# WeiZhang1988/YDORBSLAM

Measured on AMD Instinct MI355X. Metric: ORB extract+match Mkeypoints/sec, higher is better.
Workload: dtype u8

## Files before the change

ydorbslam_amd/csrc/extract_kernels.hip.h:

```cpp
#pragma once
#include <hip/hip_runtime.h>
#include <stdint.h>

#include "quadtree_core.h"
#include "quadtree_flat.h"

#pragma clang fp contract(off)

namespace ydorb {

constexpr int kPad = 19;
constexpr int kBorder = 16;
constexpr int kMaxLevels = 8;
constexpr int kTileMax = 72;
#ifndef QT_THREADS
#define QT_THREADS 512
#endif
constexpr int kQtThreads = QT_THREADS;

struct LevelDev {
  int w, h, pitch;
  int padOff;
  int blurOff, blurPitch;
  int cellBegin, nCells;
  int quota;
  int candOff;
  int kpOff;
  int tabOff;
  int nodeTabOff;
  float scale;
  float size;
};
struct PlanDev {
  int nLevels, nCellsTotal, cellCap, sumQuota;
  int maxX[16];
  unsigned nodeTabFrameStride;
  int blurTileBegin[kMaxLevels + 1];
  int borderBegin[kMaxLevels + 1];
  LevelDev lv[kMaxLevels];
};
#ifndef BLUR_TH
#define BLUR_TH 58
#endif
constexpr int kBlurTW = 64, kBlurTH = BLUR_TH;
struct CellDev {
  short level, x0, y0, x1, y1, pad0;
  int srcOff;
};

__device__ __forceinline__ int reflect101(int i, int n) {
  if (n == 1) return 0;
  while (i < 0 || i >= n) i = i < 0 ? -i : 2 * (n - 1) - i;
  return i;
}

typedef uint32_t __attribute__((aligned(1))) u32_unaligned;
typedef unsigned long long __attribute__((aligned(1))) u64_unaligned;

#ifndef PYR_ROWS
#define PYR_ROWS 8
#endif
constexpr int kPyrRows = PYR_ROWS;
__global__ __launch_bounds__(256) void k_pyr_level0(const uint8_t* __restrict__ img, int stride, size_t frameStride,
                                                    uint8_t* __restrict__ pyr, size_t pyrFrameStride, LevelDev L) {
  const int wx = blockIdx.x * 64 + (threadIdx.x & 63);
  const int yb = (blockIdx.y * 4 + __builtin_amdgcn_readfirstlane(threadIdx.x >> 6)) * kPyrRows;
  const int x0 = wx * 4 - kPad;
  if (x0 + 3 < 0 || x0 >= L.w) return;
  const uint8_t* src = img + (size_t)blockIdx.z * frameStride;
  uint8_t* dst = pyr + (size_t)blockIdx.z * pyrFrameStride + L.padOff + (size_t)kPad * L.pitch + wx * 4;
  const int xa = L.w >= 4 ? min(max(x0, 0), L.w - 4) : 0, sh = 8 * (x0 - xa);
  uint32_t v[kPyrRows];
#pragma unroll
  for (int r = 0; r < kPyrRows; r++) {
    const uint8_t* row = src + (size_t)min(yb + r, L.h - 1) * stride;
    if (L.w >= 4) {
      v[r] = *reinterpret_cast<const u32_unaligned*>(row + xa);
    } else {
      v[r] = 0;
      for (int b = 0; b < L.w; b++) v[r] |= (uint32_t)row[b] << (8 * b);
    }
    v[r] = sh < 0 ? v[r] << (-sh) : v[r] >> sh;
  }
#pragma unroll
  for (int r = 0; r < kPyrRows; r++)
    if (yb + r < L.h) *reinterpret_cast<uint32_t*>(dst + (size_t)(yb + r) * L.pitch) = v[r];
}

__global__ __launch_bounds__(256) void k_pyr_resize(uint8_t* __restrict__ pyr, size_t pyrFrameStride, LevelDev Lp, LevelDev L,
                                                    double scaleX, const short* __restrict__ alpha,
                                                    const int* __restrict__ yofs, const short* __restrict__ beta) {
  const int wx = blockIdx.x * 64 + (threadIdx.x & 63);
  const int yb = (blockIdx.y * 4 + __builtin_amdgcn_readfirstlane(threadIdx.x >> 6)) * kPyrRows;
  const int x0 = wx * 4 - kPad;
  if (x0 + 3 < 0 || x0 >= L.w) return;
  uint8_t* frame = pyr + (size_t)blockIdx.z * pyrFrameStride;
  const uint8_t* S = frame + Lp.padOff + (size_t)kPad * Lp.pitch + kPad;
  uint8_t* dst = frame + L.padOff + (size_t)kPad * L.pitch + wx * 4;
  int sx[4], sx1[4], a0[4], a1[4];
#pragma unroll
  for (int b = 0; b < 4; b++) {
    const int dx = min(max(x0 + b, 0), L.w - 1);
    const float fx = (float)__dsub_rn(__dmul_rn((double)dx + 0.5, scaleX), 0.5);
    sx[b] = min(max((int)floorf(fx), 0), Lp.w - 1);
    a0[b] = alpha[2 * dx]; a1[b] = alpha[2 * dx + 1];
    sx1[b] = min(sx[b] + 1, Lp.w - 1);
  }
  const bool fast = sx[3] - sx[0] <= 6;
  const uint8_t *r0p[kPyrRows], *r1p[kPyrRows];
  int b0[kPyrRows], b1[kPyrRows];
#pragma unroll
  for (int r = 0; r < kPyrRows; r++) {
    const int dy = min(yb + r, L.h - 1);
    const int sy = yofs[dy];
    b0[r] = beta[2 * dy]; b1[r] = beta[2 * dy + 1];
    r0p[r] = S + (size_t)min(max(sy, 0), Lp.h - 1) * Lp.pitch;
    r1p[r] = S + (size_t)min(max(sy + 1, 0), Lp.h - 1) * Lp.pitch;
  }
  uint32_t v[kPyrRows];
  if (fast) {
    typedef unsigned short u16x2 __attribute__((ext_vector_type(2)));
    uint32_t sel[4];
    u16x2 ab[4];
#pragma unroll
    for (int b = 0; b < 4; b++) {
      const uint32_t off = (uint32_t)(sx[b] - sx[0]);
      sel[b] = off | 0x0c000c00u | ((off + 1) << 16);
      ab[b] = u16x2{(unsigned short)a0[b], (unsigned short)a1[b]};
    }
    unsigned long long w0[kPyrRows], w1[kPyrRows];
#pragma unroll
    for (int r = 0; r < kPyrRows; r++) {
      w0[r] = *reinterpret_cast<const u64_unaligned*>(r0p[r] + sx[0]);
      w1[r] = *reinterpret_cast<const u64_unaligned*>(r1p[r] + sx[0]);
    }
#pragma unroll
    for (int r = 0; r < kPyrRows; r++) {
      v[r] = 0;
#pragma unroll
      for (int b = 0; b < 4; b++) {
        const uint32_t p0 = __builtin_amdgcn_perm((uint32_t)(w0[r] >> 32), (uint32_t)w0[r], sel[b]);
        const uint32_t p1 = __builtin_amdgcn_perm((uint32_t)(w1[r] >> 32), (uint32_t)w1[r], sel[b]);
        const int h0 = (int)__builtin_amdgcn_udot2(__builtin_bit_cast(u16x2, p0), ab[b], 0u, false);
        const int h1 = (int)__builtin_amdgcn_udot2(__builtin_bit_cast(u16x2, p1), ab[b], 0u, false);
        const int o = (((b0[r] * (h0 >> 4)) >> 16) + ((b1[r] * (h1 >> 4)) >> 16) + 2) >> 2;
        v[r] |= (uint32_t)(o & 0xFF) << (8 * b);
      }
    }
  } else {
#pragma unroll
    for (int r = 0; r < kPyrRows; r++) {
      v[r] = 0;
#pragma unroll
      for (int b = 0; b < 4; b++) {
        const int h0 = r0p[r][sx[b]] * a0[b] + r0p[r][sx1[b]] * a1[b];
        const int h1 = r1p[r][sx[b]] * a0[b] + r1p[r][sx1[b]] * a1[b];
        const int o = (((b0[r] * (h0 >> 4)) >> 16) + ((b1[r] * (h1 >> 4)) >> 16) + 2) >> 2;
        v[r] |= (uint32_t)(o & 0xFF) << (8 * b);
      }
    }
  }
#pragma unroll
  for (int r = 0; r < kPyrRows; r++)
    if (yb + r < L.h) *reinterpret_cast<uint32_t*>(dst + (size_t)(yb + r) * L.pitch) = v[r];
}

struct PyrPadEntry { uint32_t laneA4, laneB4, selM, selF; };
struct PyrColEntry { uint32_t sel[4]; uint32_t ab[4]; };
constexpr uint32_t kPermIdentity = 0x03020100u;
#ifndef PYR_ROWS_F
#define PYR_ROWS_F 8
#endif
constexpr int kPyrRowsF = PYR_ROWS_F;

__device__ __forceinline__ uint32_t pyr_finish_dword(uint32_t v, const PyrPadEntry& pe) {
  const uint32_t A = (uint32_t)__builtin_amdgcn_ds_bpermute((int)pe.laneA4, (int)v);
  const uint32_t B = (uint32_t)__builtin_amdgcn_ds_bpermute((int)pe.laneB4, (int)v);
  const uint32_t M = __builtin_amdgcn_perm(A, B, pe.selM);
  return __builtin_amdgcn_perm(M, v, pe.selF);
}
__device__ __forceinline__ void pyr_store_rows(uint8_t* dst, int pitch, int y, int h, uint32_t v) {
  if (y >= h) return;
  *reinterpret_cast<uint32_t*>(dst + (ptrdiff_t)y * pitch) = v;
  if (y >= 1 && y <= kPad) *reinterpret_cast<uint32_t*>(dst - (ptrdiff_t)y * pitch) = v;
  if (y >= h - 1 - kPad && y <= h - 2) *reinterpret_cast<uint32_t*>(dst + (ptrdiff_t)(2 * (h - 1) - y) * pitch) = v;
}

__global__ __launch_bounds__(256) void k_pyr_level0_f(const uint8_t* __restrict__ img, int stride, size_t frameStride,
                                                      uint8_t* __restrict__ pyr, size_t pyrFrameStride, LevelDev L,
                                                      const PyrPadEntry* __restrict__ padTab, int shift) {
  const int wx = blockIdx.x * 64 + (threadIdx.x & 63) - shift;
  const int yb = (blockIdx.y * 4 + __builtin_amdgcn_readfirstlane(threadIdx.x >> 6)) * kPyrRowsF;
  const int nd = (L.w + 2 * kPad + 3) >> 2;
  if (wx < 0 || wx >= nd) return;
  const int x0 = wx * 4 - kPad;
  const uint8_t* src = img + (size_t)blockIdx.z * frameStride;
  uint8_t* dst = pyr + (size_t)blockIdx.z * pyrFrameStride + L.padOff + (size_t)kPad * L.pitch + wx * 4;
// ... 794 lines not shown
#pragma unroll
      for (int jj = 0; jj < 4; jj++) { key[jj] = (int)(st[4 * g + jj] & 0xFFFu); slot[jj] = qf_off(Pn) + (key[jj] >> (2 * (D - Pn))); }
      for (int d = Pn - 1; d >= 1; d--) {
        const int off = qf_off(d), sh = 2 * (D - d);
#pragma unroll
        for (int jj = 0; jj < 4; jj++) {
          const int sl = off + (key[jj] >> sh);
          if (hist[sl] == 1) slot[jj] = sl;
        }
      }
#pragma unroll
      for (int jj = 0; jj < 4; jj++) st[4 * g + jj] = (st[4 * g + jj] & 0xFFFF0000u) | (uint32_t)slot[jj];
    }
  }
  if (!pairs) {
    const int TQ = ((1 << (2 * Pn)) - 1) / 3;
    const int per = (TQ + NT - 1) / NT;
    constexpr int MAXQ = ((1 << (2 * D)) - 1) / 3 / NT + 1;
    uint2 qv[MAXQ];
    int qslot[MAXQ];
    unsigned flags = 0, cntF = 0;
#pragma unroll
    for (int t = 0; t < MAXQ; t++) {
      qslot[t] = -1; qv[t] = make_uint2(0, 0);
      const int q = tid * per + t;
      if (t < per && q < TQ) {
        int d = Pn, start = 0;
        while (q >= start + (1 << (2 * (d - 1)))) { start += 1 << (2 * (d - 1)); d--; }
        const int pq = q - start;
        const int bq = pq ^ (int)(qt_flat_mask(d) >> 2);
        qslot[t] = qf_off(d) + 4 * bq;
        qv[t] = *reinterpret_cast<const QT_LDS uint2*>(hist + qslot[t]);
        const unsigned c[4] = {qv[t].x & 0xFFFFu, qv[t].x >> 16, qv[t].y & 0xFFFFu, qv[t].y >> 16};
        const unsigned sum = c[0] + c[1] + c[2] + c[3];
#pragma unroll
        for (int e = 0; e < 4; e++) {
          const unsigned cn = c[3 - e];
          const bool fl = sum >= 2 && (d == Pn ? cn >= 1 : cn == 1);
          flags |= (unsigned)fl << (4 * t + e);
          cntF += fl;
        }
      }
    }
    unsigned total;
    unsigned pos = block_scan_excl(cntF, &total);
    if ((int)total != K) { give_up(); return; }
#pragma unroll
    for (int t = 0; t < MAXQ; t++) {
      if (qslot[t] >= 0) {
        const unsigned c[4] = {qv[t].x & 0xFFFFu, qv[t].x >> 16, qv[t].y & 0xFFFFu, qv[t].y >> 16};
        unsigned o[4];
#pragma unroll
        for (int e = 0; e < 4; e++) {
          const unsigned cn = c[3 - e];
          unsigned v = 0x7FFFu;
          if ((flags >> (4 * t + e)) & 1u) {
            if ((int)pos < nOut) {
              v = pos | (cn > 16 ? 0x8000u : 0u);
              if (cn > 16) nodeBig[pos] = 1;
            }
            pos++;
          }
          o[3 - e] = v;
        }
        *reinterpret_cast<QT_LDS uint2*>(hist + qslot[t]) = make_uint2(o[0] | (o[1] << 16), o[2] | (o[3] << 16));
      }
    }
  }
  __syncthreads();

#pragma unroll
  for (int g = 0; g < ITEMS / 4; g++) {
    if (4 * g * NT < n) {
      unsigned pv[4];
#pragma unroll
      for (int jj = 0; jj < 4; jj++) pv[jj] = pairs ? st[4 * g + jj] & 0x7FFFu : hist[st[4 * g + jj] & 0xFFFFu] & 0x7FFFu;
#pragma unroll
      for (int jj = 0; jj < 4; jj++) {
        const int i = (4 * g + jj) * NT + tid;
        const bool ok = i < n && (int)pv[jj] < nOut;
        const unsigned k = ok ? pv[jj] : (unsigned)(quotaMax + 1);
        const uint32_t rs = st[4 * g + jj] & 0xFFFF0000u;
        __hip_atomic_fetch_max(nodeLo + k, ok ? rs | (0xFFFFu - (uint32_t)i) : 0u, __ATOMIC_RELAXED, __HIP_MEMORY_SCOPE_WORKGROUP);
        __hip_atomic_fetch_max(nodeHi + k, ok ? rs | (uint32_t)i : 0u, __ATOMIC_RELAXED, __HIP_MEMORY_SCOPE_WORKGROUP);
        st[4 * g + jj] = rs | (ok ? k : 0xFFFFu);
      }
    }
  }
  __syncthreads();
  for (int k = tid; k < nOut; k += NT) {
    const unsigned iLo = 0xFFFFu - (nodeLo[k] & 0xFFFFu), iHi = nodeHi[k] & 0xFFFFu;
    if (iLo == iHi || !nodeBig[k]) {
      outKp[k] = fetch((int)iLo);
    } else {
      const int s = atomicAdd(&sTieN, 1);
      if (s < kQfMaxTied) { sTieNode[s] = k; nodeBig[k] = (uint8_t)(2 + s); }
    }
  }
  __syncthreads();
  const int nTied = sTieN;
  if (nTied > kQfMaxTied) { give_up(); return; }
  if (nTied > 0) {
    const int slotCap = kQfTieCap / nTied;
    QT_LDS uint32_t* tKey = (QT_LDS uint32_t*)smem;
    QT_LDS uint32_t* tVal = tKey + kQfTieCap;
#pragma unroll
    for (int j = 0; j < ITEMS; j++) {
      if (j * NT < n) {
        const unsigned k = st[j] & 0xFFFFu;
        if (k != 0xFFFFu) {
          const unsigned tb = nodeBig[k];
          if (tb >= 2) {
            const int s = (int)tb - 2, idx = atomicAdd(&sTieCnt[s], 1);
            if (idx < slotCap) { tKey[s * slotCap + idx] = (uint32_t)(j * NT + tid); tVal[s * slotCap + idx] = st[j] >> 16; }
            else sFlag = 1;
          }
        }
      }
    }
    __syncthreads();
    if (sFlag) { give_up(); return; }
    for (int s = 0; s < nTied; s++) {
      const int m = sTieCnt[s];
      constexpr int MAXM = (kQfTieCap + NT - 1) / NT;
      int rk[MAXM];
      uint32_t oi[MAXM], rr[MAXM];
#pragma unroll
      for (int t = 0; t < MAXM; t++) {
        rk[t] = -1; oi[t] = 0; rr[t] = 0;
        const int e = tid + NT * t;
        if (e < m) {
          oi[t] = tKey[s * slotCap + e];
          rr[t] = tVal[s * slotCap + e];
          int r = 0;
          for (int u = 0; u < m; u++) r += tKey[s * slotCap + u] < oi[t];
          rk[t] = r;
        }
      }
      __syncthreads();
#pragma unroll
      for (int t = 0; t < MAXM; t++)
        if (rk[t] >= 0) { tKey[s * slotCap + rk[t]] = (rr[t] << 16) | (uint32_t)rk[t]; tVal[s * slotCap + rk[t]] = oi[t]; }
      __syncthreads();
    }
    if (tid < nTied) {
      const int m = sTieCnt[tid];
      const int best = qt_sort_front(tKey + tid * slotCap, m);
      outKp[sTieNode[tid]] = fetch((int)tVal[tid * slotCap + best]);
    }
  }
  if (tid == 0) { needPass[unit] = 0; lvlCount[unit] = nOut; }
}

__global__ __launch_bounds__(256) void k_blur(const uint8_t* __restrict__ pyr, size_t pyrFrameStride, uint8_t* __restrict__ blur,
                                              size_t blurFrameStride, PlanDev P) {
  constexpr int TW = kBlurTW, TH = kBlurTH, SH = TH + 6, SWW = 18;
  __shared__ uint32_t src[SH * SWW];
  __shared__ __align__(16) uint32_t hb[(SH / 2) * TW];
  int f = blockIdx.y, tileId = blockIdx.x;
  if ((f | 7) < (int)gridDim.y) {
    tileId = (f & 7) * (gridDim.x >> 3) + (blockIdx.x >> 3);
    f = (f & ~7) | (blockIdx.x & 7);
  }
  if (tileId >= P.blurTileBegin[P.nLevels]) return;
  int level = 0;
#pragma unroll
  for (int l = 1; l < kMaxLevels; l++)
    if (l < P.nLevels && tileId >= P.blurTileBegin[l]) level = l;
  tileId -= P.blurTileBegin[level];
  const LevelDev L = P.lv[level];
  const int tilesX = (L.w + TW - 1) / TW;
  const int ty = tileId / tilesX, tx = tileId - ty * tilesX;
  const int x0 = tx * TW, y0 = ty * TH;
  const uint8_t* padded = pyr + (size_t)f * pyrFrameStride + L.padOff;
  {
    const int r0 = threadIdx.x / SWW, wd = threadIdx.x - r0 * SWW;
    const int pcol = x0 + 16 + 4 * wd;
    const bool colOk = pcol < L.pitch;
    if (r0 < 14)
#pragma unroll
      for (int r = r0; r < SH; r += 14) {
        const int prow = min(y0 + r + kPad - 3, L.h + 2 * kPad - 1);
        src[r * SWW + wd] = colOk ? *reinterpret_cast<const uint32_t*>(padded + (size_t)prow * L.pitch + pcol) : 0u;
      }
  }
  __syncthreads();
  for (int task = threadIdx.x; task < (SH / 2) * (TW / 4); task += 256) {
    const int rp = task >> 4, g = task & 15;
    uint32_t o[2][4];
#pragma unroll
    for (int h = 0; h < 2; h++) {
      const int r = 2 * rp + h;
      const uint32_t w0 = src[r * SWW + g], w1 = src[r * SWW + g + 1], w2 = src[r * SWW + g + 2];
#pragma unroll
      for (int k = 0; k < 4; k++) {
        const uint32_t lo4 = k ? __builtin_amdgcn_alignbyte(w1, w0, k) : w0, hi4 = k ? __builtin_amdgcn_alignbyte(w2, w1, k) : w1;
        o[h][k] = __builtin_amdgcn_udot4(hi4, 0x00122230u, __builtin_amdgcn_udot4(lo4, 0x38302212u, 0u, false), false);
      }
    }
    *reinterpret_cast<uint4*>(&hb[rp * TW + g * 4]) =
        make_uint4(o[0][0] | (o[1][0] << 16), o[0][1] | (o[1][1] << 16), o[0][2] | (o[1][2] << 16), o[0][3] | (o[1][3] << 16));
  }
  __syncthreads();
  const int c4 = (threadIdx.x & 15) * 4;
#pragma unroll
  for (int r = threadIdx.x >> 4; r < TH; r += 16) {
    const int gy = y0 + r;
    if (!(gy < L.h && x0 + c4 < L.blurPitch)) continue;
    typedef unsigned short u16x2 __attribute__((ext_vector_type(2)));
    const bool odd = r & 1;
    const u16x2 k0 = odd ? u16x2{0, 18} : u16x2{18, 34}, k1 = odd ? u16x2{34, 48} : u16x2{48, 56};
    const u16x2 k2 = odd ? u16x2{56, 48} : u16x2{48, 34}, k3 = odd ? u16x2{34, 18} : u16x2{18, 0};
    const uint32_t* hp = &hb[(r >> 1) * TW + c4];
    const uint4 p0 = *reinterpret_cast<const uint4*>(hp), p1 = *reinterpret_cast<const uint4*>(hp + TW);
    const uint4 p2 = *reinterpret_cast<const uint4*>(hp + 2 * TW), p3 = *reinterpret_cast<const uint4*>(hp + 3 * TW);
    const uint32_t q0[4] = {p0.x, p0.y, p0.z, p0.w}, q1[4] = {p1.x, p1.y, p1.z, p1.w}, q2[4] = {p2.x, p2.y, p2.z, p2.w}, q3[4] = {p3.x, p3.y, p3.z, p3.w};
    uint32_t acc[4];
#pragma unroll
    for (int k = 0; k < 4; k++) {
      acc[k] = __builtin_amdgcn_udot2(__builtin_bit_cast(u16x2, q0[k]), k0, 32768u, false);
      acc[k] = __builtin_amdgcn_udot2(__builtin_bit_cast(u16x2, q1[k]), k1, acc[k], false);
      acc[k] = __builtin_amdgcn_udot2(__builtin_bit_cast(u16x2, q2[k]), k2, acc[k], false);
      acc[k] = __builtin_amdgcn_udot2(__builtin_bit_cast(u16x2, q3[k]), k3, acc[k], false);
    }
    const uint32_t out = (acc[0] >> 16) | ((acc[1] >> 16) << 8) | ((acc[2] >> 16) << 16) | ((acc[3] >> 16) << 24);
    *reinterpret_cast<uint32_t*>(blur + (size_t)f * blurFrameStride + L.blurOff + (size_t)gy * L.blurPitch + x0 + c4) = out;
  }
}

__device__ __forceinline__ float fast_atan2_deg(float y, float x) {
  const float p1 = 0.9997878412794807f * (float)(180 / 3.14159265358979323846);
  const float p3 = -0.3258083974640975f * (float)(180 / 3.14159265358979323846);
  const float p5 = 0.1555786518463281f * (float)(180 / 3.14159265358979323846);
  const float p7 = -0.04432655554792128f * (float)(180 / 3.14159265358979323846);
  const float eps = (float)2.2204460492503131e-16;
  const float ax = fabsf(x), ay = fabsf(y);
  float a, c, c2;
  if (ax >= ay) {
    c = __fdiv_rn(ay, __fadd_rn(ax, eps));
    c2 = __fmul_rn(c, c);
    a = __fmul_rn(__fadd_rn(__fmul_rn(__fadd_rn(__fmul_rn(__fadd_rn(__fmul_rn(p7, c2), p5), c2), p3), c2), p1), c);
  } else {
    c = __fdiv_rn(ax, __fadd_rn(ay, eps));
    c2 = __fmul_rn(c, c);
    a = __fsub_rn(90.f, __fmul_rn(__fadd_rn(__fmul_rn(__fadd_rn(__fmul_rn(__fadd_rn(__fmul_rn(p7, c2), p5), c2), p3), c2), p1), c));
  }
  if (x < 0) a = __fsub_rn(180.f, a);
  if (y < 0) a = __fsub_rn(360.f, a);
  return a;
}

__device__ __forceinline__ void sincos_det(float xf, float* sinOut, float* cosOut) {
  const double x = (double)xf;
  const double n = rint(__dmul_rn(x, 6.36619772367581382433e-01));
  const double r = __dsub_rn(__dsub_rn(x, __dmul_rn(n, 1.57079632673412561417e+00)), __dmul_rn(n, 6.07710050650619224932e-11));
  const double z = __dmul_rn(r, r);
  double p = __dmul_rn(z, 1.58969099521155010221e-10);
  p = __dadd_rn(p, -2.50507602534068634195e-08); p = __dmul_rn(p, z);
  p = __dadd_rn(p, 2.75573137070700676789e-06);  p = __dmul_rn(p, z);
  p = __dadd_rn(p, -1.98412698298579493134e-04); p = __dmul_rn(p, z);
  p = __dadd_rn(p, 8.33333333332248946124e-03);  p = __dmul_rn(p, z);
  p = __dadd_rn(p, -1.66666666666666324348e-01); p = __dmul_rn(p, z);
  p = __dmul_rn(p, r); p = __dadd_rn(p, r);
  double q = __dmul_rn(z, -1.13596475577881948265e-11);
  q = __dadd_rn(q, 2.08757232129817482790e-09);  q = __dmul_rn(q, z);
  q = __dadd_rn(q, -2.75573143513906633035e-07); q = __dmul_rn(q, z);
  q = __dadd_rn(q, 2.48015872894767294178e-05);  q = __dmul_rn(q, z);
  q = __dadd_rn(q, -1.38888888888741095749e-03); q = __dmul_rn(q, z);
  q = __dadd_rn(q, 4.16666666666666019037e-02);  q = __dmul_rn(q, z);
  q = __dmul_rn(q, z);
  double h = __dmul_rn(z, 0.5);
  h = __dsub_rn(h, q);
  h = __dsub_rn(1.0, h);
  const int quad = ((int)n) & 3;
  const double sv = quad == 0 ? p : quad == 1 ? h : quad == 2 ? -p : -h;
  const double cv = quad == 0 ? h : quad == 1 ? -p : quad == 2 ? -h : p;
  *sinOut = (float)sv;
  *cosOut = (float)cv;
}

__device__ __align__(16) const float kPatternDev[1024] = {
#include "orb_pattern_data.inc"
};

struct YdKeyPointDev { float x, y, size, angle, response; int octave, class_id; };

__global__ __launch_bounds__(256) void k_orient_describe(const uint8_t* __restrict__ pyr, size_t pyrFrameStride,
                                                         const uint8_t* __restrict__ blur, size_t blurFrameStride, PlanDev P,
                                                         const uint32_t* __restrict__ lvlKp, const int* __restrict__ lvlCount,
                                                         YdKeyPointDev* __restrict__ kps, uint8_t* __restrict__ desc, int cap,
                                                         int* __restrict__ nOut, float* __restrict__ lvlAngle) {
  const int lane = threadIdx.x & 63;
  int bx = blockIdx.x, f = blockIdx.y;
  if ((f | 7) < (int)gridDim.y) {
    bx = (f & 7) * (gridDim.x >> 3) + (blockIdx.x >> 3);
    f = (f & ~7) | (blockIdx.x & 7);
  }
  const int slot = bx * 4 + __builtin_amdgcn_readfirstlane(threadIdx.x >> 6);
  if (slot >= P.sumQuota) return;
  float4 pat[4];
#pragma unroll
  for (int t = 0; t < 4; t++) pat[t] = reinterpret_cast<const float4*>(kPatternDev)[t * 64 + lane];
  int level = 0;
#pragma unroll
  for (int l = 1; l < kMaxLevels; l++)
    if (l < P.nLevels && slot >= P.lv[l].kpOff) level = l;
  const uint32_t pk = __builtin_amdgcn_readfirstlane(lvlKp[(size_t)f * P.sumQuota + slot]);
  int before = 0, tot = 0, mine = 0;
#pragma unroll
  for (int l = 0; l < kMaxLevels; l++) {
    const int c = l < P.nLevels ? lvlCount[f * kMaxLevels + l] : 0;
    if (l < level) before += c;
    if (l == level) mine = c;
    tot += c;
  }
  if (slot == 0 && lane == 0) nOut[f] = min(tot, cap);
  const LevelDev L = P.lv[level];
  const int k = slot - L.kpOff;
  if (k >= mine) return;
  const int outIdx = before + k;
  if (outIdx >= cap) return;
  const int kx = qt_x(pk) + kBorder, ky = qt_y(pk) + kBorder;
  const uint8_t* roi = pyr + (size_t)f * pyrFrameStride + L.padOff + (size_t)kPad * L.pitch + kPad;
  const uint8_t* org = roi + (ptrdiff_t)(ky - 15) * L.pitch + (kx - 32);
  const int u = lane - 32;
  unsigned narrow = 0;
#pragma unroll
  for (int v = 1; v <= 15; v++) narrow |= (unsigned)(P.maxX[v] == 0) << v;
  int m10 = 0, m01 = 0;
  if (u >= -15 && u <= 15) m10 = u * org[(unsigned)(15 * L.pitch + lane)];
  if (lane >= 1 && lane <= 15 && ((narrow >> lane) & 1u)) {
    const int pos = org[(unsigned)((15 + lane) * L.pitch + 32)], neg = org[(unsigned)((15 - lane) * L.pitch + 32)];
    m01 = lane * (pos - neg);
  }
#pragma unroll
  for (int v = 1; v <= 15; v++) {
    const int d = P.maxX[v];
    if (d > 0 && u >= -d && u <= d) {
      const int pos = org[(unsigned)((15 + v) * L.pitch + lane)], neg = org[(unsigned)((15 - v) * L.pitch + lane)];
      m01 += v * (pos - neg);
      m10 += u * (pos + neg);
    }
  }
#pragma unroll
  for (int o = 32; o >= 1; o >>= 1) {
    m10 += __shfl_xor(m10, o, 64);
    m01 += __shfl_xor(m01, o, 64);
  }
  const float angle = fast_atan2_deg((float)m01, (float)m10);
  const float rad = __fmul_rn(angle, (float)(3.14159265358979323846 / 180.0));
  float sinB, cosA;
  sincos_det(rad, &sinB, &cosA);
  constexpr int kBias = 24;
  const uint8_t* bl = blur + (size_t)f * blurFrameStride + L.blurOff + (ptrdiff_t)(ky - kBias) * L.blurPitch + (kx - kBias);
  unsigned long long words[4];
#pragma unroll
  for (int t = 0; t < 4; t++) {
    const float4 pt = pat[t];
    const int r0 = __float2int_rn(__fadd_rn(__fmul_rn(pt.x, sinB), __fmul_rn(pt.y, cosA)));
    const int c0 = __float2int_rn(__fsub_rn(__fmul_rn(pt.x, cosA), __fmul_rn(pt.y, sinB)));
    const int r1 = __float2int_rn(__fadd_rn(__fmul_rn(pt.z, sinB), __fmul_rn(pt.w, cosA)));
    const int c1 = __float2int_rn(__fsub_rn(__fmul_rn(pt.z, cosA), __fmul_rn(pt.w, sinB)));
    const int t0 = bl[(unsigned)((r0 + kBias) * L.blurPitch + c0 + kBias)], t1 = bl[(unsigned)((r1 + kBias) * L.blurPitch + c1 + kBias)];
    words[t] = __ballot(t0 < t1);
  }
  if (lane < 4) {
    unsigned long long w = lane == 0 ? words[0] : lane == 1 ? words[1] : lane == 2 ? words[2] : words[3];
    reinterpret_cast<unsigned long long*>(desc + ((size_t)f * cap + outIdx) * 32)[lane] = w;
  }
  if (lane == 0) {
    YdKeyPointDev kp;
    kp.x = (float)kx;
    kp.y = (float)ky;
    if (level) { kp.x = __fmul_rn(kp.x, L.scale); kp.y = __fmul_rn(kp.y, L.scale); }
    kp.size = L.size;
    kp.angle = angle;
    kp.response = (float)qt_r(pk);
    kp.octave = level;
    kp.class_id = -1;
    kps[(size_t)f * cap + outIdx] = kp;
// ... 157 lines not shown
```

ydorbslam_amd/csrc/orb_extractor.hip:

```cpp
#include <hip/hip_runtime.h>
#include <cstdlib>

#include <algorithm>
#include <cmath>
#include <cstdarg>
#include <cstdio>
#include <cstring>
#include <string>
#include <vector>

#include "../../include/ydorb/c_api.h"
#include "extract_kernels.hip.h"
#include "host_buffers.h"
#include "ydorb_host.h"

using namespace ydorb;

namespace {

inline int cvRoundF(float v) { return (int)lrintf(v); }
inline int cvFloorF(float v) { int i = (int)v; return i - (i > v); }
inline int alignUp(int v, int a) { return (v + a - 1) / a * a; }
inline size_t alignUpZ(size_t v, size_t a) { return (v + a - 1) / a * a; }

// ... 323 lines not shown
size_t fastGeom(const HostPlan& P, int la, int lb, FastLds& fl, bool& narrow) {
  int dim = 1;
  for (int l = la; l < lb; l++) dim = std::max(dim, P.levelCellDim[l]);
  const int maxT = dim + 6, maxB = dim;
  narrow = maxT <= 44;
  const int pitch = narrow ? 48 : 80;
  fl.tileBytes = alignUp((maxT + 3) * pitch, 16);
  fl.scoreBytes = alignUp((maxB + 2) * (maxB + 2) + 4, 16);
  fl.listBytes = alignUp(2 * maxB * maxB, 16);
  return (size_t)4 * (fl.tileBytes + fl.scoreBytes + fl.listBytes);
}

template <class T> void copyTable(T* dst, const std::vector<T>& v) { if (!v.empty()) memcpy(dst, v.data(), sizeof(T) * v.size()); }

int ensurePlan(ydorb_extractor* e, int w, int h, int nFrames) {
  if (e->planValid && e->plan.w == w && e->plan.h == h && nFrames <= e->batchCap) return YDORB_OK;
  int rc = syncStreams(e);
  if (rc) return rc;
  HostPlan P;
  if ((rc = buildPlan(e, w, h, P))) return rc;
  release(e);
  const size_t B = std::max(nFrames, std::max(1, e->cfg.max_batch));
  const PlanDev& D = P.dev;
  std::vector<uint8_t> hTables(layTables(P, nullptr, e->tab));
  if ((rc = e->tables.alloc(hTables.size())) || (rc = e->work.alloc(layWork(P, B, nullptr, e->d))) ||
      (rc = e->hSync.alloc(sizeof(int) * (kMaxLevels + 2)))) return rc;
  layWork(P, B, e->work.p, e->d);
  e->h_lvlMaxN = e->hSync.as<int>();
  e->h_status = e->h_lvlMaxN + kMaxLevels + 1;
  memset(e->hSync.p, 0, e->hSync.cap);
  TablePtrs ht;
  layTables(P, hTables.data(), ht);
  copyTable(ht.cells, P.cells); copyTable(ht.tabInt, P.tabInt); copyTable(ht.tabShort, P.tabShort);
  copyTable(ht.padTab, P.padTab); copyTable(ht.colTab, P.colTab); copyTable(ht.rowTab, P.rowTab);
  layTables(P, e->tables.p, e->tab);
  if (!hTables.empty()) HIPCHK(hipMemcpyAsync(e->tables.p, hTables.data(), hTables.size(), hipMemcpyHostToDevice, e->stream));
  HIPCHK(hipMemsetAsync(e->d.pyr, 0, P.pyrFrameStride * B, e->stream));
  HIPCHK(hipMemsetAsync(e->d.needPass, 0, (uint8_t*)(e->d.passList + 1) - e->d.needPass, e->stream));
  HIPCHK(hipStreamSynchronize(e->stream));
  e->plan = P;
  e->batchCap = (int)B;
  e->imgBytes = (size_t)w * h;
  {
    FastLds fl; bool narrow;
    const size_t dynAll = fastGeom(P, 0, D.nLevels, fl, narrow);
    if (dynAll > 48 * 1024) {
      HIPCHK(hipFuncSetAttribute(reinterpret_cast<const void*>(k_fast_cells<48>), hipFuncAttributeMaxDynamicSharedMemorySize, (int)dynAll));
      HIPCHK(hipFuncSetAttribute(reinterpret_cast<const void*>(k_fast_cells<80>), hipFuncAttributeMaxDynamicSharedMemorySize, (int)dynAll));
    }
  }
  if (std::max(P.qtLdsMax, P.qtPassLds) > 48 * 1024)
  {
    HIPCHK(hipFuncSetAttribute(reinterpret_cast<const void*>(k_quadtree), hipFuncAttributeMaxDynamicSharedMemorySize, (int)std::max(P.qtLdsMax, P.qtPassLds)));
    HIPCHK(hipFuncSetAttribute(reinterpret_cast<const void*>(k_quadtree_list), hipFuncAttributeMaxDynamicSharedMemorySize, (int)std::max(P.qtLdsMax, P.qtPassLds)));
  }
  {
    int qmax = 1, tabLen = 2;
    for (int l = 0; l < D.nLevels; l++) { qmax = std::max(qmax, D.lv[l].quota); tabLen = std::max(tabLen, std::max(D.lv[l].w - 2 * kBorder, 0) + std::max(D.lv[l].h - 2 * kBorder, 0) + 2); }
    const size_t ldsFast = std::min<size_t>(qt_fast_lds_bytes(qmax, tabLen), 150 * 1024);
    if (ldsFast > 48 * 1024) {
      HIPCHK(hipFuncSetAttribute(reinterpret_cast<const void*>(k_qt_fast<8>), hipFuncAttributeMaxDynamicSharedMemorySize, (int)ldsFast));
      HIPCHK(hipFuncSetAttribute(reinterpret_cast<const void*>(k_qt_fast<16>), hipFuncAttributeMaxDynamicSharedMemorySize, (int)ldsFast));
      HIPCHK(hipFuncSetAttribute(reinterpret_cast<const void*>(k_qt_fast<32>), hipFuncAttributeMaxDynamicSharedMemorySize, (int)ldsFast));
    }
  }
  e->planValid = true;
  return YDORB_OK;
}

int ensureIo(ydorb_extractor* e) {
  if (e->io.p && e->hIo.p) return YDORB_OK;
  const size_t bytes = layIo(e->imgBytes, e->sumQuota, e->batchCap, nullptr, e->dIo);
  int rc;
  if ((rc = e->io.alloc(bytes)) || (rc = e->hIo.alloc(bytes))) return rc;
  layIo(e->imgBytes, e->sumQuota, e->batchCap, e->io.p, e->dIo);
  layIo(e->imgBytes, e->sumQuota, e->batchCap, e->hIo.p, e->hIoAt);
  return YDORB_OK;
}

void collectProfile(ydorb_extractor* e);

static void retuneQuadtree(ydorb_extractor* e) {
  HostPlan& P = e->plan;
  for (int l = 0; l < P.dev.nLevels; l++) {
    const int seen = e->h_lvlMaxN[l];
    if (seen > 0) P.qt[l].items = qfItemsFor((long)seen + seen / 8 + 32);
  }
}

int enqueue(ydorb_extractor* e, const uint8_t* d_img, int stride, size_t frameStride, int nFrames, YdKeyPointDev* d_kps,
            uint8_t* d_desc, int cap, int* d_nOut, hipStream_t s) {
  retuneQuadtree(e);
  const HostPlan& P = e->plan;
  const PlanDev& D = P.dev;
  const bool prof = e->profiling;
  if (prof) {
    if (e->profPending && hipEventQuery(e->ev[ST_COUNT]) == hipSuccess) collectProfile(e);
    e->profPending = false;
    HIPCHK(hipEventRecord(e->ev[0], s));
  }
  {
    const LevelDev& L0 = D.lv[0];
    auto fusedGrid = [&](const LevelDev& L, int shift) {
      return dim3((((L.w + 2 * kPad + 3) >> 2) + shift + 63) / 64, (L.h + 4 * kPyrRowsF - 1) / (4 * kPyrRowsF), nFrames);
    };
    if (P.fused[0].on) {
      hipLaunchKernelGGL(k_pyr_level0_f, fusedGrid(L0, P.fused[0].shift), dim3(256), 0, s, d_img, stride, frameStride, e->d.pyr, P.pyrFrameStride, L0,
                         e->tab.padTab + P.fused[0].padOff, P.fused[0].shift);
    } else {
      dim3 g((L0.pitch / 4 + 63) / 64, (L0.h + 4 * kPyrRows - 1) / (4 * kPyrRows), nFrames);
      hipLaunchKernelGGL(k_pyr_level0, g, dim3(256), 0, s, d_img, stride, frameStride, e->d.pyr, P.pyrFrameStride, L0);
    }
    for (int l = 1; l < D.nLevels; l++) {
      const LevelDev& L = D.lv[l];
      const double scaleX = 1. / ((double)L.w / D.lv[l - 1].w);
      if (P.fused[l].on) {
        const HostPlan::FusedLevel& F = P.fused[l];
        hipLaunchKernelGGL(k_pyr_resize_f, fusedGrid(L, F.shift), dim3(256), 0, s, e->d.pyr, P.pyrFrameStride, D.lv[l - 1], L, scaleX,
                           e->tab.colTab + F.colOff, e->tab.padTab + F.padOff, e->tab.rowTab + F.rowOff, F.shift);
      } else {
        dim3 gl((L.pitch / 4 + 63) / 64, (L.h + 4 * kPyrRows - 1) / (4 * kPyrRows), nFrames);
        hipLaunchKernelGGL(k_pyr_resize, gl, dim3(256), 0, s, e->d.pyr, P.pyrFrameStride, D.lv[l - 1], L, scaleX,
                           e->tab.tabShort + P.tab[l].alpha, e->tab.tabInt + P.tab[l].yofs, e->tab.tabShort + P.tab[l].beta);
      }
    }
    if (D.borderBegin[D.nLevels] > 0)
      hipLaunchKernelGGL(k_pyr_borders, dim3(D.borderBegin[D.nLevels] / 256, nFrames), dim3(256), 0, s, e->d.pyr, P.pyrFrameStride, D);
  }
  if (prof) HIPCHK(hipEventRecord(e->ev[1], s));
  hipEvent_t fastEv[kMaxLevels]{};
  int grpFirst[kMaxLevels]{}, grpEnd[kMaxLevels]{}, nGroups = 0;
  {
    const int thr = std::min(std::max(e->cfg.ini_fast_thr, 0), 255);
    int l0 = 0;
    for (int g = 0; g < e->fastGroups && l0 < D.nLevels; g++) {
      const int l1 = g == e->fastGroups - 1 ? D.nLevels : l0 + 1;
      const int c0 = D.lv[l0].cellBegin, c1 = D.lv[l1 - 1].cellBegin + D.lv[l1 - 1].nCells;
      if (c1 > c0 && D.nCellsTotal > 0) {
        FastLds fl; bool narrow;
        const size_t dyn = fastGeom(P, l0, l1, fl, narrow);
        const dim3 grid(((c1 - c0 + 3) / 4 + 7) / 8 * 8, nFrames);
        if (narrow) hipLaunchKernelGGL(k_fast_cells<48>, grid, dim3(256), dyn, s, e->d.pyr, P.pyrFrameStride, D, e->tab.cells, c0, c1, thr, fl, e->d.cellCount, e->d.cellCand);
        else hipLaunchKernelGGL(k_fast_cells<80>, grid, dim3(256), dyn, s, e->d.pyr, P.pyrFrameStride, D, e->tab.cells, c0, c1, thr, fl, e->d.cellCount, e->d.cellCand);
      }
      HIPCHK(hipEventRecord(e->evFast[l0], s));
      fastEv[l0] = e->evFast[l0];
      grpFirst[nGroups] = l0; grpEnd[nGroups] = l1; nGroups++;
      for (int l = l0 + 1; l < l1; l++) fastEv[l] = e->evFast[l0];
      l0 = l1;
    }
  }
  if (prof) HIPCHK(hipEventRecord(e->ev[2], s));
  HIPCHK(hipEventRecord(e->evFork, s));
  hipLaunchKernelGGL(k_blur, dim3((D.blurTileBegin[D.nLevels] + 7) / 8 * 8, nFrames), dim3(256), 0, s, e->d.pyr, P.pyrFrameStride, e->d.blur,
                     P.blurFrameStride, D);
  if (prof) HIPCHK(hipEventRecord(e->ev[3], s));
  bool anyFast = false;
  for (int g = 0; g < nGroups; g++) {
    const int l0 = grpFirst[g], l1 = grpEnd[g];
    const hipStream_t qs = e->qtInline ? s : e->qtStream[g % kMaxLevels];
    if (!e->qtInline) HIPCHK(hipStreamWaitEvent(qs, fastEv[l0] ? fastEv[l0] : e->evFork, 0));
    int items = 8, qmax = 1, tabLen = 2;
    for (int l = l0; l < l1; l++) {
      items = std::max(items, P.qt[l].items); qmax = std::max(qmax, D.lv[l].quota);
      tabLen = std::max(tabLen, std::max(D.lv[l].w - 2 * kBorder, 0) + std::max(D.lv[l].h - 2 * kBorder, 0) + 2);
    }
    const size_t lds = qt_fast_lds_bytes(qmax, tabLen);
    if (!e->forcePassQuadtree && lds <= 150 * 1024) {
      const dim3 grid(nFrames, l1 - l0);
#define YD_QT_FAST(IT) hipLaunchKernelGGL(k_qt_fast<IT>, grid, dim3(kQfThreads), lds, qs, D, e->d.cellCount, e->d.cellCand, l0, qmax, tabLen, e->d.lvlKp, \
                                          e->d.lvlCount, e->d.needPass, e->d.lvlMaxN, e->d.passList, e->d.passList + 1)
      if (items <= 8) YD_QT_FAST(8);
      else if (items <= 16) YD_QT_FAST(16);
      else YD_QT_FAST(32);
#undef YD_QT_FAST
      anyFast = true;
    } else {
      for (int l = l0; l < l1; l++) {
        const HostPlan::QtLevel& Q = P.qt[l];
        hipLaunchKernelGGL(k_quadtree, dim3(1, nFrames), dim3(kQtThreads), Q.lds, qs, D, e->d.cellCount, e->d.cellCand, e->d.qtCand, e->d.qtNode,
                           P.qtFrameStride, Q.nodeCap, Q.candCap, l, e->d.lvlKp, e->d.lvlCount, e->d.status, e->d.nodeScratch);
      }
    }
    if (!e->qtInline) HIPCHK(hipEventRecord(e->evJoin[g], qs));
  }
  if (!e->qtInline) for (int g = 0; g < nGroups; g++) HIPCHK(hipStreamWaitEvent(s, e->evJoin[g], 0));
  if (anyFast) {
    const int seen = e->h_lvlMaxN[kMaxLevels];
    const int listGrid = std::max(1, std::min({kQtPassWorkgroups, D.nLevels * nFrames, seen + seen / 4}));
    hipLaunchKernelGGL(k_quadtree_list, dim3(listGrid), dim3(kQtListThreads), P.qtPassLds, s, D, e->d.cellCount, e->d.cellCand,
                       e->d.qtCand, e->d.qtNode, P.qtFrameStride, -std::max(P.qtPassNodes, 1), e->d.lvlKp, e->d.lvlCount, e->d.status, e->d.passList,
                       e->d.passList + 1, e->d.nodeScratch, e->d.lvlMaxN + kMaxLevels);
    HIPCHK(hipMemsetAsync(e->d.passList, 0, sizeof(int), s));
  }
  if (prof) HIPCHK(hipEventRecord(e->ev[4], s));
  {
    const int kpw = e->descKpw;
    const dim3 gd(((D.sumQuota + 4 * kpw - 1) / (4 * kpw) + 7) / 8 * 8, nFrames);
#define YD_DESC(K) hipLaunchKernelGGL((k_orient_describe_n<K>), gd, dim3(256), 0, s, e->d.pyr, P.pyrFrameStride, e->d.blur, P.blurFrameStride, D, \
                                         e->d.lvlKp, e->d.lvlCount, d_kps, d_desc, cap, d_nOut, e->d.lvlAngle)
    if (kpw == 1)
      hipLaunchKernelGGL(k_orient_describe, gd, dim3(256), 0, s, e->d.pyr, P.pyrFrameStride, e->d.blur,
                         P.blurFrameStride, D, e->d.lvlKp, e->d.lvlCount, d_kps, d_desc, cap, d_nOut, e->d.lvlAngle);
    else if (kpw == 2) YD_DESC(2);
    else YD_DESC(4);
#undef YD_DESC
  }
  if (prof) { HIPCHK(hipEventRecord(e->ev[5], s)); e->profPending = true; }
  HIPCHK(hipMemcpyAsync(e->h_lvlMaxN, e->d.lvlMaxN, sizeof(int) * (kMaxLevels + 1), hipMemcpyDeviceToHost, s));
  HIPCHK(hipGetLastError());
  e->lastFrames = nFrames;
  e->lastStream = s;
  return YDORB_OK;
}

int checkStatus(ydorb_extractor* e) {
  if (*e->h_status == 1) { set_error("more than 65535 FAST candidates in one pyramid level"); return YDORB_ERR_CAPACITY; }
  if (*e->h_status == 3) { set_error("a pyramid level needs the pass quad-tree kernel (more candidates than LDS slots, or a very deep tree) but its quota is too large for that kernel's LDS node table"); return YDORB_ERR_CAPACITY; }
  if (*e->h_status) { set_error("quad-tree node table overflow (status %d)", *e->h_status); return YDORB_ERR_CAPACITY; }
  return YDORB_OK;
}

void collectProfile(ydorb_extractor* e) {
  if (!e->profiling || !e->profPending) return;
  e->profPending = false;
  for (int i = 0; i < ST_COUNT; i++) {
    float ms = 0;
    if (hipEventElapsedTime(&ms, e->ev[i], e->ev[i + 1]) == hipSuccess) e->stageMs[i] += ms;
  }
  e->stageCalls++;
}

}

int ydorb::extractor_pyramid_view(const ydorb_extractor* e, PyramidView* v) {
  if (!e || !v || !e->planValid || e->lastFrames < 1) { set_error("the extractor holds no pyramid (no call yet)"); return YDORB_ERR_INVALID_ARG; }
  v->device = e->cfg.device; v->nLevels = e->cfg.n_levels; v->frames = e->lastFrames; v->frameStride = (long long)e->plan.pyrFrameStride;
  v->stream = e->stream;
  for (int l = 0; l < e->cfg.n_levels; l++) {
    const LevelDev& L = e->plan.dev.lv[l];
    v->roi[l] = e->d.pyr + L.padOff + (size_t)kPad * L.pitch + kPad;
    v->w[l] = L.w; v->h[l] = L.h; v->pitch[l] = L.pitch;
    v->scale[l] = e->sf[l]; v->invScale[l] = e->isf[l];
    v->quota[l] = e->perLevel[l];
  }
  return YDORB_OK;
}

extern "C" {

int ydorb_extractor_create(const YdExtractorConfig* cfg, ydorb_extractor_t** out) {
  if (!cfg || !out) { set_error("null argument"); return YDORB_ERR_INVALID_ARG; }
  *out = nullptr;
  if (cfg->n_levels < 1 || cfg->n_levels > kMaxLevels || cfg->n_features < 1 || !(cfg->scale_factor > 1.0f)) {
    set_error("unsupported extractor config (n_levels 1..8, n_features >= 1, scale_factor > 1)");
    return YDORB_ERR_INVALID_ARG;
  }
  int rc = ydorb::require_device(cfg->device);
  if (rc) return rc;
  ydorb_extractor* e = new ydorb_extractor();
  e->cfg = *cfg;
  if (const char* v = getenv("YDORB_QT_PASS")) e->forcePassQuadtree = v[0] == '1';
  if (const char* v = getenv("YDORB_PYR_FUSED")) e->noFusedPads = v[0] == '0';
  e->descKpw = cfg->max_batch <= 8 ? 1 : 4;
  if (const char* v = getenv("YDORB_DESC_KPW")) e->descKpw = atoi(v) == 1 ? 1 : atoi(v) == 4 ? 4 : 2;
  e->cfg.min_fast_thr = cfg->ini_fast_thr;
  const int L = cfg->n_levels;
  const float s = cfg->scale_factor;
  int per = (int)round(cfg->n_features * (1 - 1.0 / s) / (1.0 - pow(1.0 / s, L)));
  int sum = 0;
  for (int i = 0; i < L; i++) {
    e->sf.push_back((float)pow(s, i));
    e->sf2.push_back((float)pow(s, 2 * i));
    e->isf.push_back((float)pow(s, -i));
    e->isf2.push_back((float)pow(s, -2 * i));
    if (i < L - 1) {
      e->perLevel.push_back(per);
      sum += per;
      per = (int)round((float)per / s);
    } else {
      e->perLevel.push_back(std::max(cfg->n_features - sum, 0));
    }
  }
  e->sumQuota = 0;
  for (int q : e->perLevel) e->sumQuota += q;
  {
    const int half = 15;
    std::vector<int> mx(half + 1, 0);
    const int maxY = (int)floor(half * sqrt(2.0) / 2.0 + 1.0), minY = (int)ceil(half * sqrt(2.0) / 2.0);
    for (int v = 0; v <= maxY; v++) mx.push_back((int)round(sqrt((double)half * half + (double)v * v)));
    for (int v = half, i = 0; v >= minY; v--) {
      while (mx[i] == mx[i + 1]) i++;
      mx[v] = i;
      i++;
    }
    for (int v = 0; v < 16; v++) e->maxX[v] = mx[v];
  }
  if (hipStreamCreateWithFlags(&e->stream, hipStreamNonBlocking) != hipSuccess) {
    set_error("hipStreamCreate failed");
    delete e;
    return YDORB_ERR_HIP;
  }
  for (auto& ev : e->ev) (void)hipEventCreate(&ev);
  (void)hipEventCreateWithFlags(&e->evFork, hipEventDisableTiming);
  for (int l = 0; l < kMaxLevels; l++) {
    const char* qtEnv = getenv("YDORB_QT_STREAMS");
    e->qtInline = (qtEnv && atoi(qtEnv) == 0) || (cfg->flags & YDORB_EXTRACTOR_SINGLE_STREAM);
    const int nQt = std::max(1, std::min(qtEnv ? atoi(qtEnv) : (cfg->max_batch <= 8 ? (int)kMaxLevels : 2), (int)kMaxLevels));
// ... 261 lines not shown
```

Baseline: 182.8.

## Compute Gaussian blur with int8 MFMA matrix ops, one tile per wavefront

```diff
diff --git a/ydorbslam_amd/csrc/extract_kernels.hip.h b/ydorbslam_amd/csrc/extract_kernels.hip.h
--- a/ydorbslam_amd/csrc/extract_kernels.hip.h
+++ b/ydorbslam_amd/csrc/extract_kernels.hip.h
@@ -39,10 +39,8 @@
   int borderBegin[kMaxLevels + 1];
   LevelDev lv[kMaxLevels];
 };
-#ifndef BLUR_TH
-#define BLUR_TH 58
-#endif
-constexpr int kBlurTW = 64, kBlurTH = BLUR_TH;
+constexpr int kBlurTW = 56, kBlurTH = 58;
+constexpr int kBlurTilesPerWg = 4;
 struct CellDev {
   short level, x0, y0, x1, y1, pad0;
   int srcOff;
@@ -1143,16 +1141,95 @@
   if (tid == 0) { needPass[unit] = 0; lvlCount[unit] = nOut; }
 }
 
-__global__ __launch_bounds__(256) void k_blur(const uint8_t* __restrict__ pyr, size_t pyrFrameStride, uint8_t* __restrict__ blur,
-                                              size_t blurFrameStride, PlanDev P) {
-  constexpr int TW = kBlurTW, TH = kBlurTH, SH = TH + 6, SWW = 18;
-  __shared__ uint32_t src[SH * SWW];
-  __shared__ __align__(16) uint32_t hb[(SH / 2) * TW];
-  int f = blockIdx.y, tileId = blockIdx.x;
+struct BlurTabs {
+  uint32_t kx[4][64][4];
+  uint32_t ky[64][2];
+};
+constexpr uint32_t blurTap(int d) { return d == 0 || d == 6 ? 18u : d == 1 || d == 5 ? 34u : d == 2 || d == 4 ? 48u : d == 3 ? 56u : 0u; }
+constexpr BlurTabs makeBlurTabs() {
+  BlurTabs T{};
+  for (int l = 0; l < 64; l++) {
+    const int n = l & 15, g = l >> 4;
+    for (int r = 0; r < 4; r++) {
+      for (int b = 0; b < 4; b++)
+        for (int t = 0; t < 4; t++) T.kx[b][l][t] |= blurTap(16 * g + 4 * t + r - (16 * (n >> 2) + 4 * b + (n & 3))) << (8 * r);
+      for (int d = 0; d < 2; d++) T.ky[l][d] |= blurTap(16 * d + 4 * g + r - n) << (8 * r);
+    }
+  }
+  return T;
+}
+__device__ __align__(16) const BlurTabs kBlurTabs = makeBlurTabs();
+
+typedef int blur_v4i __attribute__((ext_vector_type(4)));
+typedef blur_v4i __attribute__((aligned(8))) blur_v4i_a8;
+
+template <bool FULL>
+__device__ __forceinline__ void blur_tile(const uint8_t* __restrict__ src, const uint8_t* __restrict__ src0, int pitch, bool pieceOk, int rowFirst,
+                                          int rowLast, uint8_t* __restrict__ dst, int dstPitch, int rows, int cols, int lane) {
+  const int n = lane & 15, g = lane >> 4;
+  const blur_v4i zero = {0, 0, 0, 0};
+  blur_v4i a[4];
+#pragma unroll
+  for (int t = 0; t < 4; t++) {
+    const int rowOff = min(rowFirst + 16 * t + n, rowLast) * pitch;
+    if (FULL) {
+      a[t] = *reinterpret_cast<const blur_v4i_a8*>(src + rowOff);
+    } else {
+      const blur_v4i v = *reinterpret_cast<const blur_v4i_a8*>((pieceOk ? src : src0) + rowOff);
+      a[t] = pieceOk ? v : zero;
+    }
+  }
+  blur_v4i kx[4];
+#pragma unroll
+  for (int b = 0; b < 4; b++) kx[b] = *reinterpret_cast<const blur_v4i*>(&kBlurTabs.kx[b][lane][0]);
+  const uint2 kyw = *reinterpret_cast<const uint2*>(&kBlurTabs.ky[lane][0]);
+  const int ky[7] = {0, 0, 0, (int)kyw.x, (int)kyw.y, 0, 0};
+#pragma unroll
+  for (int t = 0; t < 4; t++) a[t] ^= (int)0x80808080;
+  blur_v4i ahi[4], alo[4];
+#pragma unroll
+  for (int b = 0; b < 4; b++) {
+#pragma unroll
+    for (int t = 0; t < 4; t++) {
+      const blur_v4i h = __builtin_amdgcn_mfma_i32_16x16x64_i8(a[t], kx[b], zero, 0, 0, 0);
+      const uint32_t x01 = __builtin_amdgcn_perm((uint32_t)h[1], (uint32_t)h[0], 0x05010400u);
+      const uint32_t x23 = __builtin_amdgcn_perm((uint32_t)h[3], (uint32_t)h[2], 0x05010400u);
+      alo[b][t] = (int)(__builtin_amdgcn_perm(x23, x01, 0x05040100u) ^ 0x80808080u);
+      ahi[b][t] = (int)__builtin_amdgcn_perm(x23, x01, 0x07060302u);
+    }
+  }
+  uint8_t* out = dst + (size_t)n * dstPitch + 16 * g;
+  const int left = cols - 16 * g;
+#pragma unroll
+  for (int s = 0; s < 4; s++) {
+    if (!FULL && 16 * s >= rows) return;
+    const blur_v4i kys = {ky[3 - s], ky[4 - s], ky[5 - s], ky[6 - s]};
+    uint32_t o[4];
+#pragma unroll
+    for (int b = 0; b < 4; b++) {
+      const blur_v4i zhi = __builtin_amdgcn_mfma_i32_16x16x64_i8(ahi[b], kys, zero, 0, 0, 0);
+      const blur_v4i zlo = __builtin_amdgcn_mfma_i32_16x16x64_i8(alo[b], kys, blur_v4i{8454144, 8454144, 8454144, 8454144}, 0, 0, 0);
+      uint32_t v[4];
+#pragma unroll
+      for (int r = 0; r < 4; r++) v[r] = ((uint32_t)zhi[r] << 8) + (uint32_t)zlo[r];
+      o[b] = __builtin_amdgcn_perm(v[1], v[0], 0x0c0c0602u) | __builtin_amdgcn_perm(v[3], v[2], 0x06020c0cu);
+    }
+    if (16 * s + n < rows) {
+      if (left >= 16) *reinterpret_cast<blur_v4i_a8*>(out + (size_t)(16 * s) * dstPitch) = blur_v4i{(int)o[0], (int)o[1], (int)o[2], (int)o[3]};
+      else if (left == 8) *reinterpret_cast<uint2*>(out + (size_t)(16 * s) * dstPitch) = make_uint2(o[0], o[1]);
+    }
+  }
+}
+
+__global__ __launch_bounds__(256) __attribute__((amdgpu_waves_per_eu(4))) void k_blur(const uint8_t* __restrict__ pyr, size_t pyrFrameStride,
+                                                                                      uint8_t* __restrict__ blur, size_t blurFrameStride, PlanDev P) {
+  constexpr int TW = kBlurTW, TH = kBlurTH;
+  int f = blockIdx.y, wgTile = blockIdx.x;
   if ((f | 7) < (int)gridDim.y) {
-    tileId = (f & 7) * (gridDim.x >> 3) + (blockIdx.x >> 3);
+    wgTile = (f & 7) * (gridDim.x >> 3) + (blockIdx.x >> 3);
     f = (f & ~7) | (blockIdx.x & 7);
   }
+  int tileId = kBlurTilesPerWg * wgTile + __builtin_amdgcn_readfirstlane(threadIdx.x >> 6);
   if (tileId >= P.blurTileBegin[P.nLevels]) return;
   int level = 0;
 #pragma unroll
@@ -1163,60 +1240,15 @@
   const int tilesX = (L.w + TW - 1) / TW;
   const int ty = tileId / tilesX, tx = tileId - ty * tilesX;
   const int x0 = tx * TW, y0 = ty * TH;
-  const uint8_t* padded = pyr + (size_t)f * pyrFrameStride + L.padOff;
-  {
-    const int r0 = threadIdx.x / SWW, wd = threadIdx.x - r0 * SWW;
-    const int pcol = x0 + 16 + 4 * wd;
-    const bool colOk = pcol < L.pitch;
-    if (r0 < 14)
-#pragma unroll
-      for (int r = r0; r < SH; r += 14) {
-        const int prow = min(y0 + r + kPad - 3, L.h + 2 * kPad - 1);
-        src[r * SWW + wd] = colOk ? *reinterpret_cast<const uint32_t*>(padded + (size_t)prow * L.pitch + pcol) : 0u;
-      }
-  }
-  __syncthreads();
-  for (int task = threadIdx.x; task < (SH / 2) * (TW / 4); task += 256) {
-    const int rp = task >> 4, g = task & 15;
-    uint32_t o[2][4];
-#pragma unroll
-    for (int h = 0; h < 2; h++) {
-      const int r = 2 * rp + h;
-      const uint32_t w0 = src[r * SWW + g], w1 = src[r * SWW + g + 1], w2 = src[r * SWW + g + 2];
-#pragma unroll
-      for (int k = 0; k < 4; k++) {
-        const uint32_t lo4 = k ? __builtin_amdgcn_alignbyte(w1, w0, k) : w0, hi4 = k ? __builtin_amdgcn_alignbyte(w2, w1, k) : w1;
-        o[h][k] = __builtin_amdgcn_udot4(hi4, 0x00122230u, __builtin_amdgcn_udot4(lo4, 0x38302212u, 0u, false), false);
-      }
-    }
-    *reinterpret_cast<uint4*>(&hb[rp * TW + g * 4]) =
-        make_uint4(o[0][0] | (o[1][0] << 16), o[0][1] | (o[1][1] << 16), o[0][2] | (o[1][2] << 16), o[0][3] | (o[1][3] << 16));
-  }
-  __syncthreads();
-  const int c4 = (threadIdx.x & 15) * 4;
-#pragma unroll
-  for (int r = threadIdx.x >> 4; r < TH; r += 16) {
-    const int gy = y0 + r;
-    if (!(gy < L.h && x0 + c4 < L.blurPitch)) continue;
-    typedef unsigned short u16x2 __attribute__((ext_vector_type(2)));
-    const bool odd = r & 1;
-    const u16x2 k0 = odd ? u16x2{0, 18} : u16x2{18, 34}, k1 = odd ? u16x2{34, 48} : u16x2{48, 56};
-    const u16x2 k2 = odd ? u16x2{56, 48} : u16x2{48, 34}, k3 = odd ? u16x2{34, 18} : u16x2{18, 0};
-    const uint32_t* hp = &hb[(r >> 1) * TW + c4];
-    const uint4 p0 = *reinterpret_cast<const uint4*>(hp), p1 = *reinterpret_cast<const uint4*>(hp + TW);
-    const uint4 p2 = *reinterpret_cast<const uint4*>(hp + 2 * TW), p3 = *reinterpret_cast<const uint4*>(hp + 3 * TW);
-    const uint32_t q0[4] = {p0.x, p0.y, p0.z, p0.w}, q1[4] = {p1.x, p1.y, p1.z, p1.w}, q2[4] = {p2.x, p2.y, p2.z, p2.w}, q3[4] = {p3.x, p3.y, p3.z, p3.w};
-    uint32_t acc[4];
-#pragma unroll
-    for (int k = 0; k < 4; k++) {
-      acc[k] = __builtin_amdgcn_udot2(__builtin_bit_cast(u16x2, q0[k]), k0, 32768u, false);
-      acc[k] = __builtin_amdgcn_udot2(__builtin_bit_cast(u16x2, q1[k]), k1, acc[k], false);
-      acc[k] = __builtin_amdgcn_udot2(__builtin_bit_cast(u16x2, q2[k]), k2, acc[k], false);
-      acc[k] = __builtin_amdgcn_udot2(__builtin_bit_cast(u16x2, q3[k]), k3, acc[k], false);
-    }
-    const uint32_t out = (acc[0] >> 16) | ((acc[1] >> 16) << 8) | ((acc[2] >> 16) << 16) | ((acc[3] >> 16) << 24);
-    *reinterpret_cast<uint32_t*>(blur + (size_t)f * blurFrameStride + L.blurOff + (size_t)gy * L.blurPitch + x0 + c4) = out;
-  }
+  const int lane = threadIdx.x & 63;
+  const int pcol = x0 + kPad - 3 + 16 * (lane >> 4);
+  const uint8_t* src0 = pyr + (size_t)f * pyrFrameStride + L.padOff;
+  uint8_t* dst = blur + (size_t)f * blurFrameStride + L.blurOff + (size_t)y0 * L.blurPitch + x0;
+  const int rows = min(TH, L.h - y0), cols = min(TW, L.blurPitch - x0);
+  if (rows == TH && cols == TW && x0 + kPad - 3 + 64 <= L.pitch)
+    blur_tile<true>(src0 + pcol, src0, L.pitch, true, y0 + kPad - 3, L.h + 2 * kPad - 1, dst, L.blurPitch, rows, cols, lane);
+  else
+    blur_tile<false>(src0 + pcol, src0, L.pitch, pcol + 16 <= L.pitch, y0 + kPad - 3, L.h + 2 * kPad - 1, dst, L.blurPitch, rows, cols, lane);
 }
 
 __device__ __forceinline__ float fast_atan2_deg(float y, float x) {
diff --git a/ydorbslam_amd/csrc/orb_extractor.hip b/ydorbslam_amd/csrc/orb_extractor.hip
--- a/ydorbslam_amd/csrc/orb_extractor.hip
+++ b/ydorbslam_amd/csrc/orb_extractor.hip
@@ -499,8 +499,8 @@
   }
   if (prof) HIPCHK(hipEventRecord(e->ev[2], s));
   HIPCHK(hipEventRecord(e->evFork, s));
-  hipLaunchKernelGGL(k_blur, dim3((D.blurTileBegin[D.nLevels] + 7) / 8 * 8, nFrames), dim3(256), 0, s, e->d.pyr, P.pyrFrameStride, e->d.blur,
-                     P.blurFrameStride, D);
+  hipLaunchKernelGGL(k_blur, dim3(((D.blurTileBegin[D.nLevels] + kBlurTilesPerWg - 1) / kBlurTilesPerWg + 7) / 8 * 8, nFrames), dim3(256), 0, s,
+                     e->d.pyr, P.pyrFrameStride, e->d.blur, P.blurFrameStride, D);
   if (prof) HIPCHK(hipEventRecord(e->ev[3], s));
   bool anyFast = false;
   for (int g = 0; g < nGroups; g++) {
```

Result: no change. 182.6 (-0.1%).
